# pk17r/online_3d_reconstruction

Measured on NVIDIA B200. Metric: frames_per_sec, higher is better.
Workload: dtype u8->f64->f32

## Files before the change

online_3d_reconstruction_b200/csrc/host_tile.cuh:

```cuda
#pragma once

#include "host_bucket.cuh"
#include "tile.cuh"

namespace {

struct TvPlan {
    int ntx = 0, nty = 0;
    size_t tiles_per_frame = 0;
    double L = 0;
    bool guess_pass = false;
    std::vector<uint8_t> guess;
    int R = 0;
    double wlim(int R) const { return (double)(R + 1) / L; }
};

inline bool tv_inv3(const float* T, double inv[9]) {
    const double a = T[0], b = T[1], c = T[2], d = T[4], e = T[5], f = T[6], g = T[8], h = T[9], i = T[10];
    const double A = e * i - f * h, B = -(d * i - f * g), C = d * h - e * g;
    const double det = a * A + b * B + c * C;
    const double scale = std::fabs(a) + std::fabs(b) + std::fabs(c) + std::fabs(d) + std::fabs(e) + std::fabs(f) + std::fabs(g) +
                         std::fabs(h) + std::fabs(i);
    if (!std::isfinite(det) || !(std::fabs(det) > 1e-9 * scale * scale * scale)) return false;
    const double r = 1.0 / det;
    inv[0] = A * r; inv[1] = -(b * i - c * h) * r; inv[2] = (b * f - c * e) * r;
    inv[3] = B * r; inv[4] = (a * i - c * g) * r;  inv[5] = -(a * f - c * d) * r;
    inv[6] = C * r; inv[7] = -(a * h - b * g) * r; inv[8] = (a * e - b * d) * r;
    return true;
}

bool tv_plan(const o3r_ctx* ctx, const AParams& P, const o3r_frame* frames, int n, TvPlan& pl) {
    const o3r_params& p = ctx->p;
    if (!ctx->canon || !P.vec || P.kp_tiles != 0 || P.J != 1 || P.nx <= 0 || P.ny <= 0) return false;
    const double* Q = p.Q;
    if (Q[0] == 0.0 || Q[5] == 0.0 || Q[11] == 0.0) return false;
    pl.ntx = (P.nx + kTvW - 1) / kTvW;
    pl.nty = (P.ny + kTvH - 1) / kTvH;
    pl.tiles_per_frame = (size_t)pl.ntx * pl.nty;
    const int xlo = P.x0, xhi = P.x0 + P.nx - 1, ylo = P.bb, yhi = P.bb + P.ny - 1;
    const double tx = std::max(std::fabs(Q[0] * xlo + Q[3]), std::fabs(Q[0] * xhi + Q[3])) / std::fabs(Q[11]);
    const double ty = std::max(std::fabs(Q[5] * ylo + Q[7]), std::fabs(Q[5] * yhi + Q[7])) / std::fabs(Q[11]);
    const double w_a = Q[14] * p.min_disparity + Q[15], w_b = Q[14] * 2.0 * p.min_disparity + Q[15];
    if (!(w_a != 0.0) || !std::isfinite(w_a) || !std::isfinite(w_b) || (w_a > 0) != (w_b > 0)) return false;
    const double s_a = 1.0 / w_a, s_b = 1.0 / w_b;
    const double range = std::fabs(Q[11] * s_a) * std::sqrt(1.0 + tx * tx + ty * ty);
    double tmax = 0;
    for (int i = 0; i < n; ++i)
        for (int a = 0; a < 3; ++a) tmax = std::max(tmax, (double)std::fabs(frames[i].T[4 * a + 3]));
    if (!std::isfinite(tmax) || !std::isfinite(range)) return false;
    const double edge = (double)ctx->leaf_f * 1.001 + 16.0 * FLT_EPSILON * (tmax + range);
    pl.L = 0;
    for (int i = 0; i < n; ++i) {
        double inv[9];
        if (!tv_inv3(frames[i].T, inv)) return false;
        const double sx = std::fabs(inv[0]) + std::fabs(inv[1]) + std::fabs(inv[2]);
        const double sy = std::fabs(inv[3]) + std::fabs(inv[4]) + std::fabs(inv[5]);
        const double sz = std::fabs(inv[6]) + std::fabs(inv[7]) + std::fabs(inv[8]);
        pl.L = std::max(pl.L, std::max((sx + tx * sz) / std::fabs(Q[0]), (sy + ty * sz) / std::fabs(Q[5])) * edge);
    }
    if (!std::isfinite(pl.L) || !(pl.L > 0)) return false;
    double mn[3] = {INFINITY, INFINITY, INFINITY}, mx[3] = {-INFINITY, -INFINITY, -INFINITY};
    const float* T = frames[0].T;
    for (int c = 0; c < 8; ++c) {
        const double s = (c & 1) ? s_a : s_b;
        const double cam[3] = {(Q[0] * ((c & 2) ? xhi : xlo) + Q[3]) * s, (Q[5] * ((c & 4) ? yhi : ylo) + Q[7]) * s, Q[11] * s};
        for (int a = 0; a < 3; ++a) {
            const double w = (double)T[4 * a] * cam[0] + (double)T[4 * a + 1] * cam[1] + (double)T[4 * a + 2] * cam[2];
            mn[a] = std::min(mn[a], w); mx[a] = std::max(mx[a], w);
        }
    }
    double cells = 1;
    for (int a = 0; a < 3; ++a) cells *= std::floor((mx[a] - mn[a]) * (double)ctx->inv_f) + 1.0;
    pl.guess_pass = cells > 2147483647.0;
    return true;
}

bool tv_begin(o3r_ctx* ctx, const AParams& P, const o3r_frame* frames, int n, TvPlan& pl) {
    if (ctx->tv_off || !tv_plan(ctx, P, frames, n, pl)) return false;
    pl.guess.assign(n, (uint8_t)(ctx->tv_guess >= 0 ? ctx->tv_guess : (pl.guess_pass ? 1 : 0)));
    if (ctx->tv_R < 0) {
        const double w_need = std::fabs(ctx->p.Q[14] * 2.0 * ctx->p.min_disparity + ctx->p.Q[15]);
        ctx->tv_R = kTvMaxR;
        for (int r = 1; r <= kTvMaxR; ++r)
            if (pl.wlim(r) >= w_need) { ctx->tv_R = r; break; }
    }
    return true;
}

struct TvMisc {
    uint32_t *flags, *ticket, *dbg_cnt, *cursor, *max_cursor, *fvox;
    uint8_t *guess, *actual;
};
TvMisc tv_misc(o3r_ctx* ctx, int n) {
    uint32_t* m = ctx->tv_misc.as<uint32_t>();
    uint8_t* b = reinterpret_cast<uint8_t*>(m + 16 + n);
    return TvMisc{m, m + 1, m + 2, m + 3, m + 4, m + 16, b, b + n};
}

int tv_prepare(o3r_ctx* ctx, TvPlan& pl, int n, int chunk, size_t cap_batch) {
    pl.R = std::all_of(pl.guess.begin(), pl.guess.end(), [](uint8_t g) { return g != 0; }) ? 0 : ctx->tv_R;
    const size_t tiles_chunk = pl.tiles_per_frame * (size_t)chunk, tiles_batch = pl.tiles_per_frame * (size_t)n;
    CU(ctx->tv_tiles.ensure(3 * (tiles_chunk + 4) * 4));
    CU(ctx->tv_misc.ensure((16 + (size_t)n) * 4 + 2 * (size_t)n + 16));
    CU(ctx->bbox.ensure((size_t)n * 6 * 4));
    const size_t hard_chunk = std::min(tiles_chunk * (size_t)kTvItems, pl.tiles_per_frame ? cap_batch / n * chunk : 0);
    const size_t hard_batch = std::min(tiles_batch * (size_t)kTvItems, cap_batch);
    ctx->tv_scratch_cap = std::min(std::max(ctx->tv_scratch_cap, tiles_chunk * 256), std::max<size_t>(hard_chunk, 1));
    ctx->tv_part_cap = std::min(std::max(ctx->tv_part_cap, tiles_batch * 256), std::max<size_t>(hard_batch, 1));
    if (ctx->tv_scratch_cap >= (1ull << 32) || ctx->tv_part_cap >= (1ull << 32)) return ctx->fail(O3R_ERR_INVALID, "batch too large for the tile engine");
    CU(ctx->tv_scratch.ensure(ctx->tv_scratch_cap * sizeof(o3r_cell)));
    CU(ctx->partials.ensure(ctx->tv_part_cap * sizeof(o3r_cell)));
    const TvMisc M = tv_misc(ctx, n);
    ZERO(M.flags, (16 + (size_t)n) * 4);
    const int rc = upload_small(ctx, M.guess, pl.guess.data(), (size_t)n);
    if (rc) return rc;
    return fused_prepare(ctx, cap_batch);
}

template <int DT, int R>
int tv_launch(o3r_ctx* ctx, const AParams& P, const TvArgs& A, uint32_t n_tiles) {
    const uint32_t bit = 1u << (DT * (kTvMaxR + 1) + R);
    if (!(ctx->tv_attr & bit)) {
        CU(cudaFuncSetAttribute(k_tv<DT, R>, cudaFuncAttributeMaxDynamicSharedMemorySize, (int)tv_smem<R>()));
        cudaFuncSetAttribute(k_tv<DT, R>, cudaFuncAttributePreferredSharedMemoryCarveout, 100);
        ctx->tv_attr |= bit;
    }
    LAUNCH_N("k_tv", (k_tv<DT, R>), n_tiles, kTvThreads, tv_smem<R>(), P, A);
    return O3R_OK;
}

template <int DT>
int tv_run_chunk(o3r_ctx* ctx, const AParams& P, const TvPlan& pl, int f0, int nc, int n) {
    uint32_t* cnt = ctx->counters.as<uint32_t>();
    const TvMisc M = tv_misc(ctx, n);
    const uint32_t n_tiles = (uint32_t)(pl.tiles_per_frame * (size_t)nc);
    uint32_t* tile_cnt = ctx->tv_tiles.as<uint32_t>();
    uint32_t* tile_at = tile_cnt + (pl.tiles_per_frame * (size_t)nc + 4);
    uint32_t* tile_off = tile_at + (pl.tiles_per_frame * (size_t)nc + 4);
    ZERO(M.ticket, 4);
    ZERO(M.cursor, 4);
    ZERO(cnt + CNT_PARTCHUNK, 4);
    uint32_t* bbox = ctx->bbox.as<uint32_t>() + (size_t)f0 * 6;
    FILL(bbox, (size_t)(nc) * 24, FILL_BBOX);
    TvArgs A;
    A.frames = ctx->d_frames.as<FrameDev>() + f0;
    A.frame_pass = M.guess + f0;
    A.ntx = pl.ntx; A.nty = pl.nty; A.n_frames = nc;
    A.inv_f = ctx->inv_f; A.icx = ctx->inv_c; A.icz = ctx->inv_cz;
    A.wlim = pl.R > 0 ? pl.wlim(pl.R) : INFINITY;
    {
        int dl = -1;
        for (int d = 0; d < 256; ++d)
            if (std::fabs(ctx->p.Q[14] * d + ctx->p.Q[15]) < A.wlim) dl = d; else if (dl >= 0) break;
        A.dlim_i = dl;
    }
    A.scratch = ctx->tv_scratch.as<o3r_cell>();
    A.scratch_cap = (uint32_t)ctx->tv_scratch_cap;
    A.cursor = M.cursor;
    A.tile_cnt = tile_cnt;
    A.tile_at = tile_at;
    A.ticket = M.ticket;
    A.frame_vox = M.fvox + f0;
    A.bbox = bbox;
    A.cellbb = reinterpret_cast<int*>(cnt + CNT_CELLBB);
    A.flags = M.flags;
    A.dbg_vox = ctx->keep_frame_voxels ? ctx->vox.as<float4>() : nullptr;
    A.dbg_cnt = M.dbg_cnt;
    int rc;
    switch (pl.R) {
        case 0: rc = tv_launch<DT, 0>(ctx, P, A, n_tiles); break;
        case 1: rc = tv_launch<DT, 1>(ctx, P, A, n_tiles); break;
        case 2: rc = tv_launch<DT, 2>(ctx, P, A, n_tiles); break;
        case 3: rc = tv_launch<DT, 3>(ctx, P, A, n_tiles); break;
        default: rc = tv_launch<DT, 4>(ctx, P, A, n_tiles); break;
    }
    if (rc) return rc;
    LAUNCH(k_scan_u32, 1, kScanThreads, 0, tile_cnt, tile_off, n_tiles, cnt + CNT_PARTCHUNK);
    LAUNCH(k_tv_compact, cdiv(n_tiles, kWarps), kThreads, 0, ctx->tv_scratch.as<o3r_cell>(), tile_cnt, tile_at, tile_off, n_tiles,
           ctx->partials.as<o3r_cell>(), cnt + CNT_PART, cnt + CNT_PARTCHUNK, (uint32_t)ctx->tv_part_cap, M.cursor, M.max_cursor,
           M.flags, nc, bbox, ctx->inv_f, M.guess + f0, M.actual + f0);
    LAUNCH(k_add_u32, 1, 32, 0, cnt + CNT_PART, cnt + CNT_PARTCHUNK);
    return O3R_OK;
}

int tv_read_back(o3r_ctx* ctx, int n) {
    const TvMisc M = tv_misc(ctx, n);
    CU(cudaMemcpyAsync(ctx->h_offs + 1, M.fvox, (size_t)n * 4, cudaMemcpyDeviceToHost, ctx->st));
    CU(cudaMemcpyAsync(ctx->h_offs + n + 1, M.flags, 4, cudaMemcpyDeviceToHost, ctx->st));
    CU(cudaMemcpyAsync(ctx->h_offs + n + 2, M.max_cursor, 4, cudaMemcpyDeviceToHost, ctx->st));
    CU(cudaMemcpyAsync(ctx->h_offs + n + 3, M.actual, (size_t)n, cudaMemcpyDeviceToHost, ctx->st));
    return O3R_OK;
}

Verdict tv_verdict(o3r_ctx* ctx, TvPlan& pl, int n) {
    const uint32_t* h = ctx->h_offs;
    const uint32_t fl = h[n + 1];
    const uint8_t* actual = reinterpret_cast<const uint8_t*>(h + n + 3);
    if (fl) {
        if (trace_on()) fprintf(stderr, "[o3r trace] tile engine flags %u (R %d)\n", fl, pl.R);
        if (fl & TV_FLAG_SPACE) {
            ctx->tv_scratch_cap = std::max(ctx->tv_scratch_cap, (size_t)h[n + 2] + h[n + 2] / 4 + 1024);
            ctx->tv_part_cap = std::max(ctx->tv_part_cap, (size_t)ctx->h_counters[CNT_PART] + ctx->h_counters[CNT_PART] / 4 + 1024);
        }
        if (fl & TV_FLAG_PASS) pl.guess.assign(actual, actual + n);
        else if (fl & TV_FLAG_RANGE) {
            if (pl.R >= kTvMaxR) { ctx->tv_off = true; return Verdict::NEXT_ENGINE; }
            ctx->tv_R = pl.R + 1;
        }
        return Verdict::RERUN;
    }
    ctx->tv_guess = actual[n - 1];
    size_t total_vox = 0;
    for (int i = 0; i < n; ++i) total_vox += h[i + 1];
    if ((size_t)ctx->h_counters[CNT_PART] * 4 > total_vox && total_vox > 0) ctx->tv_off = ctx->bucket_off = true;
    return Verdict::ACCEPT;
}

}
```

online_3d_reconstruction_b200/csrc/tile.cuh:

```cuda
#pragma once
#include "bucket.cuh"
#include "common.cuh"
#include "sort.cuh"
#include "stage_a.cuh"

namespace o3r {

#ifndef O3R_TV_H
#define O3R_TV_H 32
#endif
#ifndef O3R_TV_BINS
#define O3R_TV_BINS 512
#endif
#ifndef O3R_TV_THREADS
#define O3R_TV_THREADS 256
#endif
constexpr int kTvThreads = O3R_TV_THREADS;
constexpr int kTvWarps = kTvThreads / 32;
constexpr int kTvW = 64, kTvH = O3R_TV_H;
constexpr int kTvGroupsRow = kTvW / 4;
constexpr int kTvCoreGroups = kTvGroupsRow * kTvH;
constexpr int kTvQ = kTvCoreGroups / kTvThreads;
constexpr int kTvItems = kTvW * kTvH;
constexpr int kTvBinsN = O3R_TV_BINS;
template <int R>
struct TvBins { static constexpr int value = kTvBinsN; };
constexpr int kTvHash = 2 * kTvItems;
static_assert((kTvHash & (kTvHash - 1)) == 0 && kTvHash <= 65536, "hash slots: a power of two that a 16-bit cell number covers");
constexpr int tv_log2(int v) { return v <= 1 ? 0 : 1 + tv_log2(v >> 1); }
constexpr int kTvHashShift = 32 - tv_log2(kTvHash);
constexpr int kTvMaxR = 4;
constexpr uint32_t kTvNoHash = 0xffffu;
static_assert(kTvQ * kTvThreads == kTvCoreGroups, "core groups must divide evenly");

enum { TV_FLAG_RANGE = 1u, TV_FLAG_SPACE = 2u, TV_FLAG_PASS = 4u };

template <int R>
struct TvGeom {
    static constexpr int HX = R ? 4 : 0, HY = R;
    static constexpr int NC = kTvW + 2 * HX, NR = kTvH + 2 * HY, N = NC * NR, NG = N / 4;
    static constexpr int W = 2 * R + 1, S = R * W + R;
    static constexpr size_t alias_bytes = (size_t)kTvHash * 10 > (size_t)kTvItems * 16 ? (size_t)kTvHash * 10 : (size_t)kTvItems * 16;
    static constexpr size_t plane_bytes = (R && (size_t)N * 18 > alias_bytes) ? (size_t)N * 18 : alias_bytes;
};

template <int R>
struct TvMask { typedef uint32_t type; };
template <>
struct TvMask<4> { typedef unsigned long long type; };

template <int NB, int MB>
struct TvTail {
    static_assert(NB % kTvThreads == 0, "cells per thread");
    union {
        uint16_t cnt[kTvWarps][NB + 2];
        struct { double rl[256]; float zl[256]; } lut;
        unsigned long long ml[kTvItems * MB / 8];
    } u;
    uint32_t bd[NB + 1];
    uint32_t scan[34];
    uint32_t ticket, out0, nb, nitems, nbh;
    uint16_t off[40];
    int cmin[3], cmax[3];
    uint32_t bb[6];
    uint32_t any_valid, bad;
};
template <int R>
constexpr size_t tv_smem() { return TvGeom<R>::plane_bytes + sizeof(TvTail<TvBins<R>::value, (int)sizeof(typename TvMask<R>::type)>); }

template <int R>
constexpr int tv_ctas_per_sm() {
    return (int)((size_t)233472 / (tv_smem<R>() + 1024)) < 1 ? 1 : (int)((size_t)233472 / (tv_smem<R>() + 1024)) > 4 ? 4
                                                                   : (int)((size_t)233472 / (tv_smem<R>() + 1024));
}

struct TvArgs {
    const FrameDev* frames;
    const uint8_t* frame_pass;
    int ntx, nty, n_frames;
    float inv_f, icx, icz;
    double wlim;
    int dlim_i;
    o3r_cell* scratch;
    uint32_t scratch_cap;
    uint32_t* cursor;
    uint32_t* tile_cnt;
    uint32_t* tile_at;
    uint32_t* ticket;
    uint32_t* frame_vox;
    uint32_t* bbox;
    int* cellbb;
    uint32_t* flags;
    float4* dbg_vox;
    uint32_t* dbg_cnt;
};

__device__ __forceinline__ uint32_t tv_hash(int i, int j, int k) {
    uint32_t h = (uint32_t)i * 0x9e3779b1u + (uint32_t)j * 0x85ebca77u + (uint32_t)k * 0xc2b2ae3du;
    h ^= h >> 15;
    return (h ^ (h >> 17)) & 0x7fffu;
}

template <int DT>
__device__ __forceinline__ uint32_t tv_eval4(const AParams& P, const FrameDev& F, const double* rl, const float* zl, int xb, int y,
                                             const TvArgs& A, float (&X)[4], float (&Y)[4], float (&Z)[4], bool& over) {
    uint32_t mask = 0;
    const uint8_t* row = F.disp + (size_t)y * F.disp_step;
    if (DT == O3R_DISP_U8) {
        const uint32_t w = *reinterpret_cast<const uint32_t*>(row + xb);
        if (P.use_lut) {
            const double vy = __dadd_rn(__dmul_rn(P.q[5], (double)y), P.q[7]);
#pragma unroll
            for (int j = 0; j < 4; ++j) {
                const int d = (w >> (8 * j)) & 255;
                if (d > P.thr_i) {
                    mask |= 1u << j;
                    over = over || d > A.dlim_i;
                    const double s = rl[d];
                    const double v0 = __dadd_rn(__dmul_rn(P.q[0], (double)(xb + j)), P.q[3]);
                    X[j] = __double2float_rn(__dmul_rn(v0, s));
                    Y[j] = __double2float_rn(__dmul_rn(vy, s));
                    Z[j] = zl[d];
                }
            }
        } else {
#pragma unroll
            for (int j = 0; j < 4; ++j) {
                const int d = (w >> (8 * j)) & 255;
                if (d > P.thr_i) {
                    mask |= 1u << j;
                    double hw;
                    reproject_w(P, xb + j, y, (double)d, X[j], Y[j], Z[j], hw);
                    over = over || !(fabs(hw) < A.wlim);
                }
            }
        }
    } else {
        double dv[4];
        if (DT == O3R_DISP_U16) {
            const uint2 w = *reinterpret_cast<const uint2*>(row + 2 * (size_t)xb);
            dv[0] = __ddiv_rn((double)(w.x & 0xffffu), P.div); dv[1] = __ddiv_rn((double)(w.x >> 16), P.div);
            dv[2] = __ddiv_rn((double)(w.y & 0xffffu), P.div); dv[3] = __ddiv_rn((double)(w.y >> 16), P.div);
        } else if (DT == O3R_DISP_F32) {
            const float4 w = *reinterpret_cast<const float4*>(row + 4 * (size_t)xb);
            dv[0] = (double)w.x; dv[1] = (double)w.y; dv[2] = (double)w.z; dv[3] = (double)w.w;
        } else {
            const double2 a = *reinterpret_cast<const double2*>(row + 8 * (size_t)xb);
            const double2 b = *reinterpret_cast<const double2*>(row + 8 * (size_t)xb + 16);
            dv[0] = a.x; dv[1] = a.y; dv[2] = b.x; dv[3] = b.y;
        }
#pragma unroll
        for (int j = 0; j < 4; ++j)
            if (dv[j] > P.min_disp) {
                mask |= 1u << j;
                double hw;
                reproject_w(P, xb + j, y, dv[j], X[j], Y[j], Z[j], hw);
                over = over || !(fabs(hw) < A.wlim);
            }
    }
    return mask;
}

template <int R>
struct TvLater {
    static constexpr int W = 2 * R + 1, N = R + R * W;
    __device__ static __forceinline__ constexpr int bit(int dr, int dc) { return dr == 0 ? dc - 1 : R + (dr - 1) * W + (dc + R); }
    __device__ static __forceinline__ int offset(int k, int nc) {
        if (k < R) return k + 1;
        const int q = k - R, dr = q / W;
        return (dr + 1) * nc + (q - dr * W) - R;
    }
};

__device__ __forceinline__ void tv_st4(uint32_t* m, const uint32_t (&v)[4]) { *reinterpret_cast<uint4*>(m) = make_uint4(v[0], v[1], v[2], v[3]); }
__device__ __forceinline__ void tv_st4(unsigned long long* m, const unsigned long long (&v)[4]) {
    *reinterpret_cast<ulonglong2*>(m) = make_ulonglong2(v[0], v[1]);
    *reinterpret_cast<ulonglong2*>(m + 2) = make_ulonglong2(v[2], v[3]);
}
__device__ __forceinline__ void tv_ld4(const uint32_t* m, uint32_t (&v)[4]) {
    const uint4 a = *reinterpret_cast<const uint4*>(m);
    v[0] = a.x; v[1] = a.y; v[2] = a.z; v[3] = a.w;
}
__device__ __forceinline__ void tv_ld4(const unsigned long long* m, unsigned long long (&v)[4]) {
    const ulonglong2 a = *reinterpret_cast<const ulonglong2*>(m), b = *reinterpret_cast<const ulonglong2*>(m + 2);
    v[0] = a.x; v[1] = a.y; v[2] = b.x; v[3] = b.y;
}
__device__ __forceinline__ int tv_ffs(uint32_t m) { return __ffs((int)m) - 1; }
__device__ __forceinline__ int tv_ffs(unsigned long long m) { return __ffsll((long long)m) - 1; }

__device__ __forceinline__ void tv_place(const TvArgs& A, uint32_t t, uint32_t nb, uint32_t* out0) {
    const uint32_t at = nb ? atomicAdd(A.cursor, nb) : 0u;
    A.tile_cnt[t] = nb;
    A.tile_at[t] = at;
    if (at + nb > A.scratch_cap) {
        atomicOr(A.flags, TV_FLAG_SPACE);
        *out0 = 0xffffffffu;
    } else {
        *out0 = at;
    }
}
__device__ __forceinline__ void tv_cellbb(const TvArgs& A, const int* cmin, const int* cmax, int tid) {
    if (tid < 6) {
        int* gb = A.cellbb + tid;
        const int v = tid < 3 ? cmin[tid] : cmax[tid - 3];
        if (tid < 3) { if (v < *reinterpret_cast<volatile int*>(gb)) atomicMin(gb, v); }
        else { if (v > *reinterpret_cast<volatile int*>(gb)) atomicMax(gb, v); }
    }
}

__device__ __forceinline__ uint32_t tv_block_excl_scan(uint32_t v, uint32_t* sm, uint32_t& total) {
    const int lane = threadIdx.x & 31, warp = threadIdx.x >> 5;
    uint32_t inc = v;
#pragma unroll
    for (int o = 1; o < 32; o <<= 1) {
        uint32_t t = __shfl_up_sync(kFull, inc, o);
        if (lane >= o) inc += t;
    }
    if (lane == 31) sm[warp] = inc;
    __syncthreads();
    if (warp == 0) {
        uint32_t w = lane < kTvWarps ? sm[lane] : 0u, winc = w;
#pragma unroll
        for (int o = 1; o < 32; o <<= 1) {
            uint32_t t = __shfl_up_sync(kFull, winc, o);
            if (lane >= o) winc += t;
        }
        if (lane < kTvWarps) sm[lane] = winc - w;
        if (lane == kTvWarps - 1) sm[33] = winc;
    }
    __syncthreads();
    total = sm[33];
    const uint32_t r = sm[warp] + inc - v;
    __syncthreads();
    return r;
}

template <int DT, int R>
__global__ void __launch_bounds__(kTvThreads, tv_ctas_per_sm<R>()) k_tv(AParams P, TvArgs A) {
    typedef TvGeom<R> G;
    typedef typename TvMask<R>::type M;
    extern __shared__ __align__(16) unsigned char tv_smem_raw[];
    uint16_t* const SH = reinterpret_cast<uint16_t*>(tv_smem_raw);
    float* const SX = reinterpret_cast<float*>(tv_smem_raw + (size_t)G::N * 2);
    float* const SY = SX + G::N;
    float* const SZ = SY + G::N;
    uint32_t* const SC = reinterpret_cast<uint32_t*>(SZ + G::N);
    float4* const items = reinterpret_cast<float4*>(tv_smem_raw);
    constexpr int NB = TvBins<R>::value;
    typedef TvTail<NB, (int)sizeof(M)> Tail;
    Tail& S = *reinterpret_cast<Tail*>(tv_smem_raw + G::plane_bytes);
    const int tid = threadIdx.x, lane = tid & 31, warp = tid >> 5;
    const unsigned lt = (1u << lane) - 1u;

    if (tid == 0) { S.ticket = atomicAdd(A.ticket, 1u); S.any_valid = 0u; S.bad = 0u; }
    if (tid < 3) { S.cmin[tid] = 0x7fffffff; S.cmax[tid] = (int)0x80000000; S.bb[tid] = 0xffffffffu; S.bb[3 + tid] = 0u; }
    if (P.use_lut && tid < 256) { S.u.lut.rl[tid] = P.lut_r[tid]; S.u.lut.zl[tid] = P.lut_z[tid]; }
    if (R > 0 && tid < TvLater<R ? R : 1>::N) S.off[tid] = (uint16_t)TvLater<R ? R : 1>::offset(tid, G::NC);
    __syncthreads();
    const uint32_t t = S.ticket;
    const uint32_t per_frame = (uint32_t)(A.ntx * A.nty), nt = per_frame * (uint32_t)A.n_frames;
    if (t >= nt) return;
    const int f = (int)(t / per_frame);
    const int rem = (int)(t - (uint32_t)f * per_frame);
    const int tyi = rem / A.ntx, txi = rem - tyi * A.ntx;
    const FrameDev& F = A.frames[f];
    const bool pass = A.frame_pass[f] != 0;
    const int y_org = P.bb + tyi * kTvH - G::HY, x_org = P.x0 + txi * kTvW - G::HX;

    float4 cen[kTvQ * 4];
    uint32_t cvalid = 0;
    int cmn[3] = {0x7fffffff, 0x7fffffff, 0x7fffffff}, cmx[3] = {(int)0x80000000, (int)0x80000000, (int)0x80000000};
    {
        float fmn[3] = {INFINITY, INFINITY, INFINITY}, fmx[3] = {-INFINITY, -INFINITY, -INFINITY};
        bool over = false, anyv = false;
        if (R == 0) {
#pragma unroll
            for (int q = 0; q < kTvQ; ++q) {
                const int g = tid + q * kTvThreads;
                const int cr = g / kTvGroupsRow, cg = g - cr * kTvGroupsRow;
                const int y = y_org + cr, xb = x_org + cg * 4;
                if (y < P.bb + P.ny && xb < P.x0 + P.nx) {
                    float X[4], Y[4], Z[4];
                    const uint32_t mask = tv_eval4<DT>(P, F, S.u.lut.rl, S.u.lut.zl, xb, y, A, X, Y, Z, over);
                    if (mask) {
                        const uint32_t* c = reinterpret_cast<const uint32_t*>(F.bgr + (size_t)y * F.bgr_step + 3 * (size_t)xb);
                        const uint32_t w0 = __ldg(c), w1 = __ldg(c + 1), w2 = __ldg(c + 2);
                        const uint32_t rgb[4] = {w0 & 0x00ffffffu, (w0 >> 24) | ((w1 & 0xffffu) << 8), (w1 >> 16) | ((w2 & 0xffu) << 16),
                                                 w2 >> 8};
#pragma unroll
                        for (int j = 0; j < 4; ++j)
                            if (mask & (1u << j)) {
                                float4 p;
                                xform(F.T, X[j], Y[j], Z[j], p.x, p.y, p.z);
                                p.w = __uint_as_float(rgb[j]);
                                fmn[0] = fminf(fmn[0], p.x); fmx[0] = fmaxf(fmx[0], p.x);
                                fmn[1] = fminf(fmn[1], p.y); fmx[1] = fmaxf(fmx[1], p.y);
                                fmn[2] = fminf(fmn[2], p.z); fmx[2] = fmaxf(fmx[2], p.z);
                                anyv = true;
                                if (A.dbg_vox) A.dbg_vox[atomicAdd(A.dbg_cnt, 1u)] = p;
                                p.z = __fadd_rn(p.z, 500.0f);
                                const int vi = __float2int_rd(__fmul_rn(p.x, A.icx)), vj = __float2int_rd(__fmul_rn(p.y, A.icx)),
                                          vk = __float2int_rd(__fmul_rn(p.z, A.icz));
                                cmn[0] = min(cmn[0], vi); cmx[0] = max(cmx[0], vi);
                                cmn[1] = min(cmn[1], vj); cmx[1] = max(cmx[1], vj);
                                cmn[2] = min(cmn[2], vk); cmx[2] = max(cmx[2], vk);
                                cen[q * 4 + j] = p;
                                cvalid |= 1u << (q * 4 + j);
                            }
                    }
                }
            }
        } else {
        constexpr int kRounds = (G::NG + kTvThreads - 1) / kTvThreads;
#pragma unroll 1
        for (int it = 0; it < kRounds; ++it) {
            const int g = tid + it * kTvThreads;
            if (g >= G::NG) break;
            const int lr = g / (G::NC / 4), lc = (g - lr * (G::NC / 4)) * 4;
            const int y = y_org + lr, xb = x_org + lc;
            uint2 hh = make_uint2(0xffffffffu, 0xffffffffu);
            float px[4] = {0.f, 0.f, 0.f, 0.f}, py[4] = {0.f, 0.f, 0.f, 0.f}, pz[4] = {0.f, 0.f, 0.f, 0.f};
            uint32_t rgb[4] = {0u, 0u, 0u, 0u};
            if (y >= P.bb && y < P.bb + P.ny && xb >= P.x0 && xb < P.x0 + P.nx) {
                float X[4], Y[4], Z[4];
                const uint32_t* c = reinterpret_cast<const uint32_t*>(F.bgr + (size_t)y * F.bgr_step + 3 * (size_t)xb);
                const uint32_t w0 = __ldg(c), w1 = __ldg(c + 1), w2 = __ldg(c + 2);
                const uint32_t mask = tv_eval4<DT>(P, F, S.u.lut.rl, S.u.lut.zl, xb, y, A, X, Y, Z, over);
                if (mask) {
                    rgb[0] = w0 & 0x00ffffffu;
                    rgb[1] = (w0 >> 24) | ((w1 & 0xffffu) << 8);
                    rgb[2] = (w1 >> 16) | ((w2 & 0xffu) << 16);
                    rgb[3] = w2 >> 8;
                    const bool core = lr >= G::HY && lr < G::HY + kTvH && lc >= G::HX && lc < G::HX + kTvW;
                    uint32_t h[4] = {kTvNoHash, kTvNoHash, kTvNoHash, kTvNoHash};
#pragma unroll
                    for (int j = 0; j < 4; ++j)
                        if (mask & (1u << j)) {
                            xform(F.T, X[j], Y[j], Z[j], px[j], py[j], pz[j]);
                            int ci, cj, ck;
                            bk_cell(px[j], py[j], pz[j], A.inv_f, ci, cj, ck);
                            h[j] = tv_hash(ci, cj, ck);
                            if (core) {
                                fmn[0] = fminf(fmn[0], px[j]); fmx[0] = fmaxf(fmx[0], px[j]);
                                fmn[1] = fminf(fmn[1], py[j]); fmx[1] = fmaxf(fmx[1], py[j]);
                                fmn[2] = fminf(fmn[2], pz[j]); fmx[2] = fmaxf(fmx[2], pz[j]);
                                anyv = true;
                            }
                        }
                    hh = make_uint2(h[0] | (h[1] << 16), h[2] | (h[3] << 16));
                }
            }
            const int o = lr * G::NC + lc;
            *reinterpret_cast<uint2*>(SH + o) = hh;
            *reinterpret_cast<float4*>(SX + o) = make_float4(px[0], px[1], px[2], px[3]);
            *reinterpret_cast<float4*>(SY + o) = make_float4(py[0], py[1], py[2], py[3]);
            *reinterpret_cast<float4*>(SZ + o) = make_float4(pz[0], pz[1], pz[2], pz[3]);
            *reinterpret_cast<uint4*>(SC + o) = make_uint4(rgb[0], rgb[1], rgb[2], rgb[3]);
        }
        }
        const unsigned anyw = __ballot_sync(kFull, anyv);
        if (anyw) {
            uint32_t mn[3], mx[3];
#pragma unroll
            for (int a = 0; a < 3; ++a) {
                mn[a] = __reduce_min_sync(kFull, anyv ? f2ord(fmn[a]) : 0xffffffffu);
                mx[a] = __reduce_max_sync(kFull, anyv ? f2ord(fmx[a]) : 0u);
            }
            if (lane == 0) {
                S.any_valid = 1u;
#pragma unroll
                for (int a = 0; a < 3; ++a) { atomicMin(&S.bb[a], mn[a]); atomicMax(&S.bb[3 + a], mx[a]); }
            }
        }
        if (over && !pass) S.bad = 1u;
    }
    __syncthreads();
    if (S.any_valid && tid < 6) {
        uint32_t* gb = A.bbox + (size_t)f * 6 + tid;
        const uint32_t v = S.bb[tid];
        if (tid < 3) { if (v < *reinterpret_cast<volatile uint32_t*>(gb)) atomicMin(gb, v); }
        else { if (v > *reinterpret_cast<volatile uint32_t*>(gb)) atomicMax(gb, v); }
    }
    if (tid == 0 && S.bad) atomicOr(A.flags, TV_FLAG_RANGE);

    if (R > 0 && !pass) {
        typedef TvLater<R> LW;
        M* const mlS = reinterpret_cast<M*>(&S.u);
        for (int g = tid; g < (G::HY + kTvH) * (G::NC / 4); g += kTvThreads) {
            const int lr = g / (G::NC / 4), lc = (g - lr * (G::NC / 4)) * 4;
            const int o = lr * G::NC + lc;
            const uint2 h2 = *reinterpret_cast<const uint2*>(SH + o);
            if ((h2.x & h2.y) == 0xffffffffu) {
                if (lr >= G::HY && lc >= G::HX && lc < G::HX + kTvW) {
                    const M zero[4] = {0, 0, 0, 0};
                    tv_st4(mlS + ((lr - G::HY) * kTvW + (lc - G::HX)), zero);
                }
                continue;
            }
            const uint32_t h[4] = {h2.x & 0xffffu, h2.x >> 16, h2.y & 0xffffu, h2.y >> 16};
            M ml[4] = {0, 0, 0, 0};
            const uint2 none = make_uint2(0xffffffffu, 0xffffffffu);
#pragma unroll
            for (int dr = 0; dr <= R; ++dr) {
                const uint16_t* hr = SH + (lr + dr) * G::NC + lc - 4;
                const uint2 a = (lc >= 4 && dr > 0) ? *reinterpret_cast<const uint2*>(hr) : none;
                const uint2 b = *reinterpret_cast<const uint2*>(hr + 4);
                const uint2 c = (lc + 8 <= G::NC) ? *reinterpret_cast<const uint2*>(hr + 8) : none;
                const uint32_t w[12] = {a.x & 0xffffu, a.x >> 16, a.y & 0xffffu, a.y >> 16, b.x & 0xffffu, b.x >> 16,
                                        b.y & 0xffffu, b.y >> 16, c.x & 0xffffu, c.x >> 16, c.y & 0xffffu, c.y >> 16};
#pragma unroll
                for (int j = 0; j < 4; ++j)
#pragma unroll
                    for (int dc = (dr == 0 ? 1 : -R); dc <= R; ++dc)
                        if (w[4 + j + dc] == h[j]) ml[j] |= (M)1 << LW::bit(dr, dc);
            }
#pragma unroll
            for (int j = 0; j < 4; ++j) {
                M l = h[j] == kTvNoHash ? (M)0 : ml[j], keep = 0;
                if (l) {
                    const int oc = o + j;
                    int ci, cj, ck;
                    bk_cell(SX[oc], SY[oc], SZ[oc], A.inv_f, ci, cj, ck);
                    while (l) {
                        const int k = tv_ffs(l);
                        l &= l - 1;
                        const int on = oc + (int)S.off[k];
                        int ni, nj, nk;
                        bk_cell(SX[on], SY[on], SZ[on], A.inv_f, ni, nj, nk);
                        if (ni == ci && nj == cj && nk == ck) {
                            keep |= (M)1 << k;
                            SC[on] |= 0x80000000u;
                        }
                    }
                }
                ml[j] = keep;
            }
            if (lr >= G::HY && lc >= G::HX && lc < G::HX + kTvW) tv_st4(mlS + ((lr - G::HY) * kTvW + (lc - G::HX)), ml);
        }
        __syncthreads();
        uint32_t todo = 0;
#pragma unroll
        for (int q = 0; q < kTvQ; ++q) {
            const int g = tid + q * kTvThreads;
            const int o = (g / kTvGroupsRow + G::HY) * G::NC + (g % kTvGroupsRow) * 4 + G::HX;
            const uint2 h2 = *reinterpret_cast<const uint2*>(SH + o);
            const uint4 c4 = *reinterpret_cast<const uint4*>(SC + o);
            const uint32_t hv[4] = {h2.x & 0xffffu, h2.x >> 16, h2.y & 0xffffu, h2.y >> 16}, cv[4] = {c4.x, c4.y, c4.z, c4.w};
            M mv[4];
            tv_ld4(mlS + g * 4, mv);
#pragma unroll
            for (int j = 0; j < 4; ++j)
                if (hv[j] != kTvNoHash && !(cv[j] & 0x80000000u) && mv[j] != 0) todo |= 1u << (q * 4 + j);
        }
        while (todo) {
            const int r = __ffs((int)todo) - 1;
            todo &= todo - 1;
            const int g = tid + (r >> 2) * kTvThreads;
            const int oc = (g / kTvGroupsRow + G::HY) * G::NC + (g % kTvGroupsRow) * 4 + G::HX + (r & 3);
            M l = mlS[g * 4 + (r & 3)];
            float sx = __fadd_rn(0.f, SX[oc]), sy = __fadd_rn(0.f, SY[oc]), sz = __fadd_rn(0.f, SZ[oc]);
            uint32_t w = SC[oc];
            uint32_t cn = 1, cr = (w >> 16) & 255u, cg = (w >> 8) & 255u, cb = w & 255u;
            while (l) {
                const int k = tv_ffs(l);
                l &= l - 1;
                const int on = oc + (int)S.off[k];
                sx = __fadd_rn(sx, SX[on]); sy = __fadd_rn(sy, SY[on]); sz = __fadd_rn(sz, SZ[on]);
                w = SC[on];
                cr += (w >> 16) & 255u; cg += (w >> 8) & 255u; cb += w & 255u;
                ++cn;
            }
            const float4 c = bk_centroid(sx, sy, sz, cn, cr, cg, cb);
            SX[oc] = c.x; SY[oc] = c.y; SZ[oc] = c.z; SC[oc] = __float_as_uint(c.w);
        }
        __syncthreads();
    }
    if (R > 0) {
#pragma unroll
        for (int r = 0; r < kTvQ * 4; ++r) {
            const int g = tid + (r >> 2) * kTvThreads;
            const int o = (g / kTvGroupsRow + G::HY) * G::NC + (g % kTvGroupsRow) * 4 + G::HX;
            const uint2 h2 = *reinterpret_cast<const uint2*>(SH + o);
            const uint4 c4 = *reinterpret_cast<const uint4*>(SC + o);
            const float4 x4 = *reinterpret_cast<const float4*>(SX + o), y4 = *reinterpret_cast<const float4*>(SY + o),
                         z4 = *reinterpret_cast<const float4*>(SZ + o);
            const int j = r & 3;
            const uint32_t hq = j == 0 ? (h2.x & 0xffffu) : j == 1 ? (h2.x >> 16) : j == 2 ? (h2.y & 0xffffu) : (h2.y >> 16);
            const uint32_t w = j == 0 ? c4.x : j == 1 ? c4.y : j == 2 ? c4.z : c4.w;
            if (hq == kTvNoHash || (w & 0x80000000u)) continue;
            float4 c = make_float4(j == 0 ? x4.x : j == 1 ? x4.y : j == 2 ? x4.z : x4.w, j == 0 ? y4.x : j == 1 ? y4.y : j == 2 ? y4.z : y4.w,
                                   j == 0 ? z4.x : j == 1 ? z4.y : j == 2 ? z4.z : z4.w, __uint_as_float(w));
            if (!pass) {
                c.x = __fadd_rn(0.f, c.x); c.y = __fadd_rn(0.f, c.y); c.z = __fadd_rn(0.f, c.z);
            }
            if (A.dbg_vox) A.dbg_vox[atomicAdd(A.dbg_cnt, 1u)] = c;
            c.z = __fadd_rn(c.z, 500.0f);
            const int vi = __float2int_rd(__fmul_rn(c.x, A.icx)), vj = __float2int_rd(__fmul_rn(c.y, A.icx)),
                      vk = __float2int_rd(__fmul_rn(c.z, A.icz));
            cmn[0] = min(cmn[0], vi); cmx[0] = max(cmx[0], vi);
            cmn[1] = min(cmn[1], vj); cmx[1] = max(cmx[1], vj);
            cmn[2] = min(cmn[2], vk); cmx[2] = max(cmx[2], vk);
            cen[r] = c;
            cvalid |= 1u << r;
        }
    }
    {
        const unsigned anyc = __ballot_sync(kFull, cvalid != 0u);
        if (anyc) {
#pragma unroll
            for (int a = 0; a < 3; ++a) {
                cmn[a] = __reduce_min_sync(kFull, cmn[a]);
                cmx[a] = __reduce_max_sync(kFull, cmx[a]);
            }
            if (lane == 0) {
#pragma unroll
                for (int a = 0; a < 3; ++a) { atomicMin(&S.cmin[a], cmn[a]); atomicMax(&S.cmax[a], cmx[a]); }
            }
        }
    }
    __syncthreads();
    const bool have = S.cmin[0] != 0x7fffffff;
    const int c0i = S.cmin[0], c0j = S.cmin[1], c0k = S.cmin[2];
    const long long ei = have ? (long long)S.cmax[0] - c0i + 1 : 0, ej = have ? (long long)S.cmax[1] - c0j + 1 : 0,
                    ek = have ? (long long)S.cmax[2] - c0k + 1 : 0;
    const bool fits = ei * ej * ek <= (long long)NB && ei <= NB && ej <= NB && ek <= NB;
    int nbins = fits ? (int)(ei * ej * ek) : 0;
    const int Bi = 1 << 20;
    uint32_t bin[kTvQ * 4], rk[kTvQ * 4];
#pragma unroll
    for (int r = 0; r < kTvQ * 4; ++r) bin[r] = (uint32_t)(NB + 1);
    bool loose = false;
    if (fits) {
#pragma unroll
        for (int r = 0; r < kTvQ * 4; ++r)
            if ((cvalid >> r) & 1u) {
                const int vi = __float2int_rd(__fmul_rn(cen[r].x, A.icx)), vj = __float2int_rd(__fmul_rn(cen[r].y, A.icx)),
                          vk = __float2int_rd(__fmul_rn(cen[r].z, A.icz));
                bin[r] = (uint32_t)(((vk - c0k) * (int)ej + (vj - c0j)) * (int)ei + (vi - c0i));
            }
    } else {
        unsigned long long* const tab = reinterpret_cast<unsigned long long*>(tv_smem_raw);
        uint16_t* const dense = reinterpret_cast<uint16_t*>(tv_smem_raw + (size_t)kTvHash * 8);
        {
            uint4* tz = reinterpret_cast<uint4*>(tab);
            for (int i = tid; i < kTvHash / 2; i += kTvThreads) tz[i] = make_uint4(~0u, ~0u, ~0u, ~0u);
            if (tid == 0) S.nbh = 0u;
        }
        __syncthreads();
#pragma unroll
        for (int r = 0; r < kTvQ * 4; ++r)
            if ((cvalid >> r) & 1u) {
                const int vi = __float2int_rd(__fmul_rn(cen[r].x, A.icx)), vj = __float2int_rd(__fmul_rn(cen[r].y, A.icx)),
                          vk = __float2int_rd(__fmul_rn(cen[r].z, A.icz));
                const unsigned long long k = ((unsigned long long)(uint32_t)(vk + Bi) << 42) | ((unsigned long long)(uint32_t)(vj + Bi) << 21) |
                                             (unsigned long long)(uint32_t)(vi + Bi);
                uint32_t h = ((uint32_t)(k ^ (k >> 21) ^ (k >> 42)) * 0x9e3779b1u) >> kTvHashShift;
                for (;;) {
                    const unsigned long long old = atomicCAS(&tab[h], ~0ull, k);
                    if (old == ~0ull) { dense[h] = (uint16_t)atomicAdd(&S.nbh, 1u); break; }
                    if (old == k) break;
                    h = (h + 1) & (kTvHash - 1);
                }
                bin[r] = h;
            }
        __syncthreads();
        nbins = (int)S.nbh;
        loose = nbins > NB;
        if (!loose) {
#pragma unroll
            for (int r = 0; r < kTvQ * 4; ++r)
                if ((cvalid >> r) & 1u) bin[r] = dense[bin[r]];
        }
        __syncthreads();
    }
    if (loose) {
        uint32_t tot;
        uint32_t pos = tv_block_excl_scan((uint32_t)__popc(cvalid), S.scan, tot);
        if (tid == 0) tv_place(A, t, tot, &S.out0);
        __syncthreads();
        if (tot == 0) return;
        if (tid == 0) atomicAdd(A.frame_vox + f, tot);
        tv_cellbb(A, S.cmin, S.cmax, tid);
        if (S.out0 == 0xffffffffu) return;
        o3r_cell* const out = A.scratch + S.out0;
#pragma unroll
        for (int r = 0; r < kTvQ * 4; ++r)
            if ((cvalid >> r) & 1u) {
                const float4 p = cen[r];
                const int vi = __float2int_rd(__fmul_rn(p.x, A.icx)), vj = __float2int_rd(__fmul_rn(p.y, A.icx)),
                          vk = __float2int_rd(__fmul_rn(p.z, A.icz));
                const uint32_t w = __float_as_uint(p.w);
                o3r_cell c;
                c.key = ((unsigned long long)(uint32_t)(vk + Bi) << 42) | ((unsigned long long)(uint32_t)(vj + Bi) << 21) |
                        (unsigned long long)(uint32_t)(vi + Bi);
                c.sx = p.x; c.sy = p.y; c.sz = p.z; c.n = 1u;
                c.sr = (w >> 16) & 255u; c.sg = (w >> 8) & 255u; c.sb = w & 255u; c.pad = 0u;
                out[pos++] = c;
            }
        return;
    }
    for (int b = tid; b < (nbins + 2) * kTvWarps; b += kTvThreads) {
        const int w = b / (nbins + 2), i = b - w * (nbins + 2);
        S.u.cnt[w][i == nbins + 1 ? NB + 1 : i] = 0;
    }
    __syncthreads();
    uint16_t* wc = &S.u.cnt[warp][0];
#pragma unroll
    for (int r = 0; r < kTvQ * 4; ++r) {
        const unsigned peers = __match_any_sync(kFull, bin[r]);
        const uint32_t old = wc[bin[r]];
        __syncwarp();
        if ((peers & lt) == 0u) wc[bin[r]] = (uint16_t)(old + __popc(peers));
        __syncwarp();
        rk[r] = old + __popc(peers & lt);
    }
    __syncthreads();
    {
        constexpr int BPT = NB / kTvThreads;
        uint32_t run[BPT], psum = 0;
#pragma unroll
        for (int qq = 0; qq < BPT; ++qq) {
            const int b = tid * BPT + qq;
            uint32_t acc = 0;
            if (b < nbins) {
#pragma unroll
                for (int w = 0; w < kTvWarps; ++w) { const uint32_t c = S.u.cnt[w][b]; S.u.cnt[w][b] = (uint16_t)acc; acc += c; }
            }
            run[qq] = acc | (acc ? 1u << 16 : 0u);
            psum += run[qq];
        }
        uint32_t tot;
        uint32_t ds = tv_block_excl_scan(psum, S.scan, tot);
#pragma unroll
        for (int qq = 0; qq < BPT; ++qq) {
            const int b = tid * BPT + qq;
            if (b < nbins) S.bd[b] = ds;
            ds += run[qq];
        }
        if (tid == 0) { S.bd[nbins] = tot; S.nitems = tot & 0xffffu; S.nb = tot >> 16; }
    }
    __syncthreads();
    const uint32_t nb = S.nb;
#pragma unroll
    for (int r = 0; r < kTvQ * 4; ++r)
        if ((cvalid >> r) & 1u) items[(S.bd[bin[r]] & 0xffffu) + (uint32_t)wc[bin[r]] + rk[r]] = cen[r];
    if (tid == 0) tv_place(A, t, nb, &S.out0);
    __syncthreads();
    if (nb == 0) return;
    if (tid == 0) atomicAdd(A.frame_vox + f, S.nitems);
    tv_cellbb(A, S.cmin, S.cmax, tid);
    if (S.out0 == 0xffffffffu) return;
    o3r_cell* const out = A.scratch + S.out0;
    for (int b0 = warp * 8; b0 < nbins; b0 += kTvWarps * 8) {
        const int b = b0 + (lane >> 2), sub = lane & 3;
        uint32_t a = 0, e = 0, dense = 0;
        if (b < nbins) {
            const uint32_t v0 = S.bd[b], v1 = S.bd[b + 1];
            a = v0 & 0xffffu; e = v1 & 0xffffu; dense = v0 >> 16;
        }
        float sx = 0.f, sy = 0.f, sz = 0.f;
        uint32_t cr = 0, cg = 0, cb = 0;
        for (uint32_t i = a + sub; i < e; i += 4) {
            const float4 p = items[i];
            sx = __fadd_rn(sx, p.x); sy = __fadd_rn(sy, p.y); sz = __fadd_rn(sz, p.z);
            const uint32_t w = __float_as_uint(p.w);
            cr += (w >> 16) & 255u; cg += (w >> 8) & 255u; cb += w & 255u;
        }
#pragma unroll
        for (int o = 1; o <= 2; o <<= 1) {
            sx = __fadd_rn(sx, __shfl_xor_sync(kFull, sx, o));
            sy = __fadd_rn(sy, __shfl_xor_sync(kFull, sy, o));
            sz = __fadd_rn(sz, __shfl_xor_sync(kFull, sz, o));
            cr += __shfl_xor_sync(kFull, cr, o); cg += __shfl_xor_sync(kFull, cg, o); cb += __shfl_xor_sync(kFull, cb, o);
        }
        if (sub == 0 && e > a) {
            const float4 p0 = items[a];
            const int vi = __float2int_rd(__fmul_rn(p0.x, A.icx)), vj = __float2int_rd(__fmul_rn(p0.y, A.icx)),
                      vk = __float2int_rd(__fmul_rn(p0.z, A.icz));
            o3r_cell c;
            c.key = ((unsigned long long)(uint32_t)(vk + Bi) << 42) | ((unsigned long long)(uint32_t)(vj + Bi) << 21) |
                    (unsigned long long)(uint32_t)(vi + Bi);
            c.sx = sx; c.sy = sy; c.sz = sz; c.n = e - a;
            c.sr = cr; c.sg = cg; c.sb = cb; c.pad = 0u;
            out[dense] = c;
        }
    }
}

__global__ void __launch_bounds__(kThreads) k_tv_compact(const o3r_cell* __restrict__ scratch, const uint32_t* __restrict__ tile_cnt,
                                                         const uint32_t* __restrict__ tile_at, const uint32_t* __restrict__ tile_off,
                                                         uint32_t n_tiles, o3r_cell* __restrict__ out,
                                                         const uint32_t* __restrict__ out_base, const uint32_t* __restrict__ chunk_total,
                                                         uint32_t out_cap, const uint32_t* __restrict__ cursor,
                                                         uint32_t* __restrict__ max_cursor, uint32_t* __restrict__ flags, int n_frames,
                                                         const uint32_t* __restrict__ bbox, float inv_f,
                                                         const uint8_t* __restrict__ guess, uint8_t* __restrict__ actual) {
    if (blockIdx.x == 0 && threadIdx.x == 0) atomicMax(max_cursor, *cursor);
    if (blockIdx.x == gridDim.x - 1)
        for (int f = threadIdx.x; f < n_frames; f += kThreads) {
            const GridParams G = make_grid(bbox + 6 * f, inv_f, inv_f, inv_f);
            const uint8_t a = (uint8_t)(G.passthrough ? 1 : 0);
            actual[f] = G.empty ? guess[f] : a;
            if (!G.empty && a != guess[f]) atomicOr(flags, TV_FLAG_PASS);
        }
    const bool room = (unsigned long long)*out_base + *chunk_total <= (unsigned long long)out_cap;
    if (!room && blockIdx.x == 0 && threadIdx.x == 0) atomicOr(flags, TV_FLAG_SPACE);
    if (!room || (*flags & TV_FLAG_SPACE)) return;
    const uint32_t t = blockIdx.x * kWarps + (threadIdx.x >> 5), lane = threadIdx.x & 31;
    if (t >= n_tiles) return;
    const uint32_t n = tile_cnt[t];
    if (n == 0) return;
    const unsigned long long* src = reinterpret_cast<const unsigned long long*>(scratch + tile_at[t]);
    unsigned long long* dst = reinterpret_cast<unsigned long long*>(out + *out_base + tile_off[t]);
    const uint32_t nw = n * 5u;
    uint32_t i = lane;
    for (; i + 96u < nw; i += 128u) {
        const unsigned long long a = __ldcs(src + i), b = __ldcs(src + i + 32), c = __ldcs(src + i + 64), d = __ldcs(src + i + 96);
        dst[i] = a; dst[i + 32] = b; dst[i + 64] = c; dst[i + 96] = d;
    }
    for (; i < nw; i += 32u) dst[i] = __ldcs(src + i);
}

}
```

Before: 42090.

## Move halo-pass bbox reduction out of transform loop and size scratch by tile items

Result: faster. 43260, median of 6 (+2.8%).

```diff
diff --git a/online_3d_reconstruction_b200/csrc/host_tile.cuh b/online_3d_reconstruction_b200/csrc/host_tile.cuh
--- a/online_3d_reconstruction_b200/csrc/host_tile.cuh
+++ b/online_3d_reconstruction_b200/csrc/host_tile.cuh
@@ -105,8 +105,8 @@
     CU(ctx->bbox.ensure((size_t)n * 6 * 4));
     const size_t hard_chunk = std::min(tiles_chunk * (size_t)kTvItems, pl.tiles_per_frame ? cap_batch / n * chunk : 0);
     const size_t hard_batch = std::min(tiles_batch * (size_t)kTvItems, cap_batch);
-    ctx->tv_scratch_cap = std::min(std::max(ctx->tv_scratch_cap, tiles_chunk * 256), std::max<size_t>(hard_chunk, 1));
-    ctx->tv_part_cap = std::min(std::max(ctx->tv_part_cap, tiles_batch * 256), std::max<size_t>(hard_batch, 1));
+    ctx->tv_scratch_cap = std::min(std::max(ctx->tv_scratch_cap, tiles_chunk * (kTvItems / 8)), std::max<size_t>(hard_chunk, 1));
+    ctx->tv_part_cap = std::min(std::max(ctx->tv_part_cap, tiles_batch * (kTvItems / 8)), std::max<size_t>(hard_batch, 1));
     if (ctx->tv_scratch_cap >= (1ull << 32) || ctx->tv_part_cap >= (1ull << 32)) return ctx->fail(O3R_ERR_INVALID, "batch too large for the tile engine");
     CU(ctx->tv_scratch.ensure(ctx->tv_scratch_cap * sizeof(o3r_cell)));
     CU(ctx->partials.ensure(ctx->tv_part_cap * sizeof(o3r_cell)));
diff --git a/online_3d_reconstruction_b200/csrc/tile.cuh b/online_3d_reconstruction_b200/csrc/tile.cuh
--- a/online_3d_reconstruction_b200/csrc/tile.cuh
+++ b/online_3d_reconstruction_b200/csrc/tile.cuh
@@ -8,6 +8,9 @@
 
 #ifndef O3R_TV_H
 #define O3R_TV_H 32
+#endif
+#ifndef O3R_TV_CTAS
+#define O3R_TV_CTAS 4
 #endif
 #ifndef O3R_TV_BINS
 #define O3R_TV_BINS 512
@@ -68,11 +71,13 @@
 template <int R>
 constexpr size_t tv_smem() { return TvGeom<R>::plane_bytes + sizeof(TvTail<TvBins<R>::value, (int)sizeof(typename TvMask<R>::type)>); }
 
+constexpr int kTvCtas = O3R_TV_CTAS;
 template <int R>
-constexpr int tv_ctas_per_sm() {
-    return (int)((size_t)233472 / (tv_smem<R>() + 1024)) < 1 ? 1 : (int)((size_t)233472 / (tv_smem<R>() + 1024)) > 4 ? 4
-                                                                   : (int)((size_t)233472 / (tv_smem<R>() + 1024));
-}
+constexpr int tv_smem_ctas() { return (int)((size_t)233472 / (tv_smem<R>() + 1024)); }
+template <int R>
+constexpr int tv_ctas_per_sm() { return tv_smem_ctas<R>() < 1 ? 1 : tv_smem_ctas<R>() < kTvCtas ? tv_smem_ctas<R>() : kTvCtas; }
+static_assert(tv_smem_ctas<0>() >= kTvCtas && tv_smem_ctas<1>() >= kTvCtas && tv_smem_ctas<2>() >= kTvCtas,
+              "at window radii up to 2 (configs[1] runs R = 2) the shared memory of a tile must let kTvCtas CTAs onto an SM");
 
 struct TvArgs {
     const FrameDev* frames;
@@ -161,6 +166,14 @@
     return mask;
 }
 
+__device__ __forceinline__ void tv_axis4(const float* Ta, uint32_t mask, const float (&X)[4], const float (&Y)[4], const float (&Z)[4],
+                                         float (&o)[4]) {
+    const float t0 = Ta[0], t1 = Ta[1], t2 = Ta[2], t3 = Ta[3];
+#pragma unroll
+    for (int j = 0; j < 4; ++j)
+        if (mask & (1u << j)) o[j] = __fadd_rn(__fadd_rn(__fadd_rn(__fmul_rn(t0, X[j]), __fmul_rn(t1, Y[j])), __fmul_rn(t2, Z[j])), t3);
+}
+
 template <int R>
 struct TvLater {
     static constexpr int W = 2 * R + 1, N = R + R * W;
@@ -233,6 +246,21 @@
     const uint32_t r = sm[warp] + inc - v;
     __syncthreads();
     return r;
+}
+
+__device__ __forceinline__ void tv_bbox_warp(bool anyv, const float (&fmn)[3], const float (&fmx)[3], uint32_t* bb, uint32_t* any_valid) {
+    if (!__ballot_sync(kFull, anyv)) return;
+    uint32_t mn[3], mx[3];
+#pragma unroll
+    for (int a = 0; a < 3; ++a) {
+        mn[a] = __reduce_min_sync(kFull, anyv ? f2ord(fmn[a]) : 0xffffffffu);
+        mx[a] = __reduce_max_sync(kFull, anyv ? f2ord(fmx[a]) : 0u);
+    }
+    if ((threadIdx.x & 31) == 0) {
+        *any_valid = 1u;
+#pragma unroll
+        for (int a = 0; a < 3; ++a) { atomicMin(&bb[a], mn[a]); atomicMax(&bb[3 + a], mx[a]); }
+    }
 }
 
 template <int DT, int R>
@@ -271,9 +299,10 @@
     uint32_t cvalid = 0;
     int cmn[3] = {0x7fffffff, 0x7fffffff, 0x7fffffff}, cmx[3] = {(int)0x80000000, (int)0x80000000, (int)0x80000000};
     {
-        float fmn[3] = {INFINITY, INFINITY, INFINITY}, fmx[3] = {-INFINITY, -INFINITY, -INFINITY};
-        bool over = false, anyv = false;
+        bool over = false;
         if (R == 0) {
+            float fmn[3] = {INFINITY, INFINITY, INFINITY}, fmx[3] = {-INFINITY, -INFINITY, -INFINITY};
+            bool anyv = false;
 #pragma unroll
             for (int q = 0; q < kTvQ; ++q) {
                 const int g = tid + q * kTvThreads;
@@ -310,6 +339,7 @@
                     }
                 }
             }
+            tv_bbox_warp(anyv, fmn, fmx, S.bb, &S.any_valid);
         } else {
         constexpr int kRounds = (G::NG + kTvThreads - 1) / kTvThreads;
 #pragma unroll 1
@@ -331,21 +361,16 @@
                     rgb[1] = (w0 >> 24) | ((w1 & 0xffffu) << 8);
                     rgb[2] = (w1 >> 16) | ((w2 & 0xffu) << 16);
                     rgb[3] = w2 >> 8;
-                    const bool core = lr >= G::HY && lr < G::HY + kTvH && lc >= G::HX && lc < G::HX + kTvW;
+                    tv_axis4(F.T, mask, X, Y, Z, px);
+                    tv_axis4(F.T + 4, mask, X, Y, Z, py);
+                    tv_axis4(F.T + 8, mask, X, Y, Z, pz);
                     uint32_t h[4] = {kTvNoHash, kTvNoHash, kTvNoHash, kTvNoHash};
 #pragma unroll
                     for (int j = 0; j < 4; ++j)
                         if (mask & (1u << j)) {
-                            xform(F.T, X[j], Y[j], Z[j], px[j], py[j], pz[j]);
                             int ci, cj, ck;
                             bk_cell(px[j], py[j], pz[j], A.inv_f, ci, cj, ck);
                             h[j] = tv_hash(ci, cj, ck);
-                            if (core) {
-                                fmn[0] = fminf(fmn[0], px[j]); fmx[0] = fmaxf(fmx[0], px[j]);
-                                fmn[1] = fminf(fmn[1], py[j]); fmx[1] = fmaxf(fmx[1], py[j]);
-                                fmn[2] = fminf(fmn[2], pz[j]); fmx[2] = fmaxf(fmx[2], pz[j]);
-                                anyv = true;
-                            }
                         }
                     hh = make_uint2(h[0] | (h[1] << 16), h[2] | (h[3] << 16));
                 }
@@ -358,30 +383,33 @@
             *reinterpret_cast<uint4*>(SC + o) = make_uint4(rgb[0], rgb[1], rgb[2], rgb[3]);
         }
         }
-        const unsigned anyw = __ballot_sync(kFull, anyv);
-        if (anyw) {
-            uint32_t mn[3], mx[3];
-#pragma unroll
-            for (int a = 0; a < 3; ++a) {
-                mn[a] = __reduce_min_sync(kFull, anyv ? f2ord(fmn[a]) : 0xffffffffu);
-                mx[a] = __reduce_max_sync(kFull, anyv ? f2ord(fmx[a]) : 0u);
-            }
-            if (lane == 0) {
-                S.any_valid = 1u;
-#pragma unroll
-                for (int a = 0; a < 3; ++a) { atomicMin(&S.bb[a], mn[a]); atomicMax(&S.bb[3 + a], mx[a]); }
-            }
-        }
         if (over && !pass) S.bad = 1u;
     }
     __syncthreads();
-    if (S.any_valid && tid < 6) {
-        uint32_t* gb = A.bbox + (size_t)f * 6 + tid;
-        const uint32_t v = S.bb[tid];
-        if (tid < 3) { if (v < *reinterpret_cast<volatile uint32_t*>(gb)) atomicMin(gb, v); }
-        else { if (v > *reinterpret_cast<volatile uint32_t*>(gb)) atomicMax(gb, v); }
-    }
     if (tid == 0 && S.bad) atomicOr(A.flags, TV_FLAG_RANGE);
+    if (R > 0) {
+        float fmn[3] = {INFINITY, INFINITY, INFINITY}, fmx[3] = {-INFINITY, -INFINITY, -INFINITY};
+        bool anyv = false;
+#pragma unroll
+        for (int q = 0; q < kTvQ; ++q) {
+            const int g = tid + q * kTvThreads;
+            const int o = (g / kTvGroupsRow + G::HY) * G::NC + (g % kTvGroupsRow) * 4 + G::HX;
+            const uint2 h2 = *reinterpret_cast<const uint2*>(SH + o);
+            const float4 x4 = *reinterpret_cast<const float4*>(SX + o), y4 = *reinterpret_cast<const float4*>(SY + o),
+                         z4 = *reinterpret_cast<const float4*>(SZ + o);
+            const uint32_t hv[4] = {h2.x & 0xffffu, h2.x >> 16, h2.y & 0xffffu, h2.y >> 16};
+            const float xv[4] = {x4.x, x4.y, x4.z, x4.w}, yv[4] = {y4.x, y4.y, y4.z, y4.w}, zv[4] = {z4.x, z4.y, z4.z, z4.w};
+#pragma unroll
+            for (int j = 0; j < 4; ++j)
+                if (hv[j] != kTvNoHash) {
+                    fmn[0] = fminf(fmn[0], xv[j]); fmx[0] = fmaxf(fmx[0], xv[j]);
+                    fmn[1] = fminf(fmn[1], yv[j]); fmx[1] = fmaxf(fmx[1], yv[j]);
+                    fmn[2] = fminf(fmn[2], zv[j]); fmx[2] = fmaxf(fmx[2], zv[j]);
+                    anyv = true;
+                }
+        }
+        tv_bbox_warp(anyv, fmn, fmx, S.bb, &S.any_valid);
+    }
 
     if (R > 0 && !pass) {
         typedef TvLater<R> LW;
@@ -519,6 +547,12 @@
         }
     }
     __syncthreads();
+    if (S.any_valid && tid < 6) {
+        uint32_t* gb = A.bbox + (size_t)f * 6 + tid;
+        const uint32_t v = S.bb[tid];
+        if (tid < 3) { if (v < *reinterpret_cast<volatile uint32_t*>(gb)) atomicMin(gb, v); }
+        else { if (v > *reinterpret_cast<volatile uint32_t*>(gb)) atomicMax(gb, v); }
+    }
     const bool have = S.cmin[0] != 0x7fffffff;
     const int c0i = S.cmin[0], c0j = S.cmin[1], c0k = S.cmin[2];
     const long long ei = have ? (long long)S.cmax[0] - c0i + 1 : 0, ej = have ? (long long)S.cmax[1] - c0j + 1 : 0,
```
